# google/sentencepiece

Hardware: AMD Instinct MI355X
Metric: sentences/sec EncodeBatch, 32k unigram, MI355X (higher is better)
Workload: dtype u8 text -> i32 ids; f64 add / f32 store in the Viterbi relax

## Files before the change

### sentencepiece_amd/csrc/api.cc

```cpp
#include <hip/hip_runtime.h>

#include <cstdio>
#include <cstdlib>
#include <fcntl.h>
#include <sys/mman.h>
#include <sys/stat.h>
#include <sys/syscall.h>
#include <unistd.h>

#include <algorithm>
#include <cmath>
#include <condition_variable>
#include <cstring>
#include <fstream>
#include <functional>
#include <map>
#include <memory>
#include <mutex>
#include <thread>
#include <new>
#include <sstream>
#include <atomic>
#include <chrono>
#include <string>
// ... 650 lines not shown
  HIP_OR_RETURN(h, ws->d_tmp_off.Reserve(n + 1));
  HIP_OR_RETURN(h, ws->d_tile_sums.Reserve((n + kScanTile - 1) / kScanTile + 2));
  HIP_OR_RETURN(h, ws->d_big_list.Reserve((n + 63) / 64 + 1));
  if (!d_status) { HIP_OR_RETURN(h, ws->d_sent_status.Reserve(n)); d_status = ws->d_sent_status.p; }
  uint32_t *const class_lists = ws->d_lists.p;
  uint32_t *const over_list = class_lists + static_cast<size_t>(kMaxClasses - 1) * n;
  uint32_t *const hard_lists = class_lists + static_cast<size_t>(kMaxClasses) * n;
  uint32_t *const long_list = class_lists + static_cast<size_t>(2 * kMaxClasses) * n;
  uint32_t *const retry_lists[2] = {long_list + n, long_list + 2 * n};
  uint32_t *const left_lists[3] = {long_list + 3 * n, long_list + (3 + static_cast<size_t>(kMaxClasses)) * n,
                                   long_list + (3 + 2 * static_cast<size_t>(kMaxClasses)) * n};
  uint32_t *const gen_lists = long_list + (3 + 3 * static_cast<size_t>(kMaxClasses)) * n;
  uint64_t expand = (h->dev.flags & kNfCompressSp) || !(h->dev.flags & kNfEscapeWs) ? 1 : 3;
  if ((h->dev.flags & kNfCompressSp) && (h->dev.flags & kNfByteFallback)) expand = 2;
  uint64_t arena_need = expand * text_bytes + (10 + static_cast<uint64_t>(h->dev.n_prefix + h->dev.n_suffix)) * n + 4096;
  const bool prof = h->profiling;
  if (prof) HIP_OR_RETURN(h, EnsureEvents(ws));
  const uint32_t n32 = static_cast<uint32_t>(n);
  const int wide = h->n_cu * 8;
  const bool fast_ok = StreamFastEligible(h->dev.flags) && !h->no_fast;
  const bool uds = (h->dev.flags & kNfHasUserDefined) != 0;
  uint32_t rcaps[kMaxClasses] = {0};
  for (int c = 0; c < ncls; ++c) rcaps[c] = cls[c].rcap;
  rcaps[ncls - 1] = cls[ncls - 1].rcap;
  const uint64_t max_raw = (0x7FFFFF00ull - 16) / h->dev.expand_max;
  auto record = [&](int slot, int which) -> hipError_t {
    return prof ? hipEventRecord(ws->ev[slot][which], stream) : hipSuccess;
  };
  auto scan_compact = [&]() -> int {
    ScanArgs sa{ws->d_counts.p, n32, ws->d_tile_sums.p, d_id_offsets};
    const uint32_t tiles = (n32 + kScanTile - 1) / kScanTile;
    HIP_OR_RETURN(h, LaunchScan(sa, static_cast<int>(tiles < static_cast<uint32_t>(wide) ? tiles : wide), stream));
    const uint32_t big = (n < 65536 || text_bytes > 160ull * n) ? h->compact_big : 0u;
    CompactArgs pa{ws->d_arena.p, ws->d_tmp_off.p, ws->d_counts.p, d_id_offsets, d_ids, d_ids ? ids_capacity : 0, n32, &ws->d_ctrl->status, h->compact_staged,
                   big, ws->d_big_list.p, &ws->d_ctrl->big_count[0]};
    const uint64_t cblocks = (n + 63) / 64;
    const uint64_t cgrid = cblocks < static_cast<uint64_t>(h->n_cu) * 32 ? cblocks : static_cast<uint64_t>(h->n_cu) * 32;
    HIP_OR_RETURN(h, LaunchCompact(pa, static_cast<int>(cgrid), stream));
    if (big) HIP_OR_RETURN(h, LaunchCompactBig(pa, h->n_cu * 4, stream));
    HIP_OR_RETURN(h, hipMemcpyAsync(ws->h_ctrl, ws->d_ctrl, offsetof(Ctrl, total_ids), hipMemcpyDeviceToHost, stream));
    HIP_OR_RETURN(h, hipMemcpyAsync(&ws->h_ctrl->total_ids, d_id_offsets + n, sizeof(uint64_t), hipMemcpyDeviceToHost, stream));
    HIP_OR_RETURN(h, hipStreamSynchronize(stream));
    return kOk;
  };
  uint64_t arena_cap_limit = 0;
  if (h->arena_first && arena_need > h->arena_first) { arena_need = h->arena_first; arena_cap_limit = h->arena_first; }
  const uint64_t arena_reserve = (h->arena_first || ws->reserve_text_bytes <= text_bytes) ? 0 :
      expand * ws->reserve_text_bytes + (10 + static_cast<uint64_t>(h->dev.n_prefix + h->dev.n_suffix)) * (ws->reserve_n > n ? ws->reserve_n : n) + 4096;
  for (int attempt = 0; attempt < 4; ++attempt) {
    HIP_OR_RETURN(h, ws->d_arena.Reserve(arena_need > arena_reserve ? arena_need : arena_reserve));
    if (spans) HIP_OR_RETURN(h, ws->d_arena_tb.Reserve(ws->d_arena.cap));
    if (prof) HIP_OR_RETURN(h, hipEventRecord(ws->ev[kNumSlots][0], stream));
    HIP_OR_RETURN(h, hipMemsetAsync(ws->d_ctrl, 0, sizeof(Ctrl), stream));
    HIP_OR_RETURN(h, hipMemsetAsync(d_status, 0, n, stream));
    for (bool &u : ws->slot_used) u = false;
    const bool direct = word_ok && any_word && h->word_form == 3 && !h->no_direct && streaming;
    uint32_t known[kMaxClasses] = {0};
    uint32_t gen_known[kMaxClasses] = {0};
    uint64_t gen_total = 0;
    if (!direct) {
      if (int rc = RunClassify(h, ws, d_offsets, n32, stream, scanned ? d_text : nullptr, text_bytes, scanned ? gen_lists : nullptr); rc != kOk) return rc;
      HIP_OR_RETURN(h, hipMemcpyAsync(ws->h_ctrl->list_counts, ws->d_ctrl->list_counts,
                                      sizeof(ws->h_ctrl->list_counts) + sizeof(ws->h_ctrl->gen_counts),
                                      hipMemcpyDeviceToHost, stream));
      HIP_OR_RETURN(h, hipStreamSynchronize(stream));
      for (int c = 0; c < ncls; ++c) { known[c] = ws->h_ctrl->list_counts[c]; gen_known[c] = ws->h_ctrl->gen_counts[c]; gen_total += gen_known[c]; }
    } else {
      known[0] = n32;
    }
    EncodeArgs a{};
    a.dev = h->dev; a.text = d_text; a.offs = d_offsets;
// ... 286 lines not shown
        }
        wa.total_main = tile_base;
        wa.q = &ws->d_ctrl->q[qi];
        wa.stats = &ws->d_ctrl->stats[kStatsPerClass * slot];
        wa.left_lists = out_lists;
        wa.left_counts = d_out_counts;
        wa.left2_lists = out2_lists;
        wa.left2_counts = d_out2_counts;
        wa.dyn_tag = ws->d_dyn_tag.p;
        wa.dyn_ent = ws->d_dyn_ent.p;
        wa.dyn_list = ws->d_dyn_list.p;
        wa.dyn_count = &ws->d_ctrl->dyn_count;
        wa.dyn_mask = h->dyn_slots - 1u;
        wa.dyn_cap = h->dyn_list_cap;
        wa.resume = ws->d_resume.p;
        wa.ids16 = (h->model.pieces.size() <= 65536 && !h->no_ids16) ? 1u : 0u;
        snprintf(ws->slot_name[slot], sizeof(ws->slot_name[slot]), "%s",
                 wform ? (wa.ids16 ? (mode == 2 ? "EncodeWordWaveAgainKernel<true>" : mode == 1 ? "EncodeWordWaveCollectKernel<true>" : "EncodeWordWaveKernel<true>")
                                   : (mode == 2 ? "EncodeWordWaveAgainKernel<false>" : mode == 1 ? "EncodeWordWaveCollectKernel<false>" : "EncodeWordWaveKernel<false>"))
                       : mode == 3 ? "EncodeWordDpKernel" : mode == 2 ? "EncodeWordAgainKernel" : mode == 1 ? "EncodeWordCollectKernel" : "EncodeWordKernel");
        HIP_OR_RETURN(h, record(slot, 0));
        if (wform) HIP_OR_RETURN(h, LaunchEncodeWordWave(mode, wa, static_cast<int>(grid), waves, WordWaveLdsBytes(waves), stream));
        else HIP_OR_RETURN(h, LaunchEncodeWord(mode, wa, static_cast<int>(grid), waves, WordLdsBytes(waves, dp), stream));
        HIP_OR_RETURN(h, record(slot, 1));
        ws->slot_used[slot] = true;
        return kOk;
      };
      auto read_counts = [&]() -> int {
        HIP_OR_RETURN(h, hipMemcpyAsync(ws->h_ctrl->left_counts, ws->d_ctrl->left_counts, sizeof(ws->h_ctrl->left_counts) + sizeof(uint32_t),
                                        hipMemcpyDeviceToHost, stream));
        HIP_OR_RETURN(h, hipStreamSynchronize(stream));
// ... 111 lines not shown
      Profile &p = ws->prof;
      p = Profile();
      p.n = kNumSlots;
      for (int c = 0; c < kNumSlots; ++c) {
        if (!ws->slot_used[c]) continue;
        memcpy(p.name[c], ws->slot_name[c], sizeof(p.name[c]));
        HIP_OR_RETURN(h, hipEventElapsedTime(&p.kernel_ms[c], ws->ev[c][0], ws->ev[c][1]));
        const unsigned long long *s = &ws->h_ctrl->stats[kStatsPerClass * c];
        p.sentences[c] = s[0];
        p.raw_bytes[c] = s[1];
        p.ids[c] = s[2];
        for (int k = 0; k < 5; ++k) p.cycles[c][k] = s[3 + k];
      }
      p.path[0] = ws->h_ctrl->side.n_backlog; p.path[1] = ws->h_ctrl->side.over_count; p.path[2] = ws->h_ctrl->side.long_count;
      p.path[3] = ws->h_ctrl->side.n_failed;
      HIP_OR_RETURN(h, hipEventElapsedTime(&p.total_ms, ws->ev[kNumSlots][0], ws->ev[kNumSlots][1]));
      std::lock_guard<std::mutex> l(h->mu);
      h->prof = p;
    }
    if (total_ids) *total_ids = ws->h_ctrl->total_ids;
    if (n_failed) *n_failed = ws->h_ctrl->side.n_failed;
    if (ws->h_ctrl->total_ids > ids_capacity || !d_ids) {
      if (ws->h_ctrl->total_ids == 0) return kOk;
      return Fail(h, kResourceExhausted, "ids_capacity is too small");
    }
    if (spans && ws->h_ctrl->total_ids > 0) {
      const uint64_t total = ws->h_ctrl->total_ids;
      HIP_OR_RETURN(h, ws->d_tok_begin.Reserve(total));
      CompactArgs pa{ws->d_arena_tb.p, ws->d_tmp_off.p, ws->d_counts.p, d_id_offsets, ws->d_tok_begin.p, total, n32, nullptr, h->compact_staged,
                     h->compact_big, ws->d_big_list.p, &ws->d_ctrl->big_count[1]};
      const uint64_t cblocks = (n + 63) / 64;
      const uint64_t cgrid = cblocks < static_cast<uint64_t>(h->n_cu) * 32 ? cblocks : static_cast<uint64_t>(h->n_cu) * 32;
      HIP_OR_RETURN(h, LaunchCompact(pa, static_cast<int>(cgrid), stream));
      if (h->compact_big) HIP_OR_RETURN(h, LaunchCompactBig(pa, h->n_cu * 4, stream));
      HIP_OR_RETURN(h, hipMemsetAsync(&ws->d_ctrl->status, 0, sizeof(uint32_t), stream));
      HIP_OR_RETURN(h, hipMemsetAsync(ws->d_ctrl->align_counts, 0, sizeof(ws->d_ctrl->align_counts), stream));
      HIP_OR_RETURN(h, hipMemsetAsync(&ws->d_ctrl->side.long_count, 0, sizeof(uint32_t), stream));
      AlignArgs base{};
      base.dev = h->dev; base.text = d_text; base.offs = d_offsets;
      base.id_offs = d_id_offsets; base.tok_begin = ws->d_tok_begin.p; base.begin = d_begin; base.end = d_end;
      base.nbegin = d_nbegin; base.nend = d_nbegin ? d_nend : nullptr;
      base.status = &ws->d_ctrl->status; base.list_cap = n32;
      bool prev = false;
      int c_staged = 0;
      while (c_staged < ncls && cls[c_staged].rcap <= kMaxStagedRaw) ++c_staged;
// ... 1694 lines not shown
  snprintf(out, cap, "%s", h->prof.name[slot]);
  return static_cast<int>(strlen(h->prof.name[slot]));
}

int spmx_last_profile(const spmx_handle *h, float *kernel_ms, uint64_t *sentences, uint64_t *raw_bytes, uint64_t *ids,
                      uint64_t *bytes, uint64_t *path, float *total_ms) {
  if (!h) return 0;
  const Profile &p = h->prof;
  for (int c = 0; c < p.n; ++c) {
    if (kernel_ms) kernel_ms[c] = p.kernel_ms[c];
    if (sentences) sentences[c] = p.sentences[c];
    if (raw_bytes) raw_bytes[c] = p.raw_bytes[c];
    if (ids) ids[c] = p.ids[c];
    if (bytes) bytes[c] = p.raw_bytes[c] + 16 * p.sentences[c] + 4 * p.ids[c];
  }
  if (path) for (int k = 0; k < 4; ++k) path[k] = p.path[k];
  if (total_ms) *total_ms = p.total_ms;
  return p.n;
}

}
```

### sentencepiece_amd/csrc/kernels.h

```cpp
#ifndef SPMX_KERNELS_H_
#define SPMX_KERNELS_H_

#ifndef SPMX_WAVE_API
#include "wave.h"
#endif
#include <math.h>

#include "dev.h"

namespace spmx {

enum : uint32_t {
  kStArenaOverflow = 1u << 0,
  kStTooLong = 1u << 1,
  kStInternal = 1u << 2,
};
enum : uint32_t { kSsOk = 0, kSsResourceExhausted = 8, kSsOutOfRange = 11, kSsInternal = 13 };

constexpr int kMaxClasses = 8;

struct StreamClass {
  uint32_t rcap;
  uint32_t tcap;
  uint32_t lane_shift;
// ... 53 lines not shown
  uint32_t no_char_norm;
  StreamClass cls[kMaxClasses];
  uint32_t *left_lists;
  uint32_t *left_counts;
  uint32_t *left2_lists;
  uint32_t *left2_counts;
  unsigned long long *dyn_tag;
  U4 *dyn_ent;
  uint32_t *dyn_list;
  uint32_t *dyn_count;
  uint32_t dyn_mask;
  uint32_t dyn_cap;
  U4 *resume;
  uint32_t ids16;
  uint32_t direct;
  const uint32_t *list;
  const uint32_t *list_count;
  uint32_t *next_list;
  uint32_t *next_count;
  uint32_t rcap, ncap;
};

constexpr int kStatsPerClass = 8;
constexpr uint32_t kTokEnd = 0x8000u;

SPMX_DEVICE uint32_t DartsOffset(uint32_t u) { return (u >> 10) << ((u & (1u << 9)) >> 6); }

SPMX_DEVICE int OneCharLenDev(uint32_t c) {
  const uint32_t h = c >> 4;
  return h < 12 ? 1 : (h < 14 ? 2 : (h == 14 ? 3 : 4));
// ... 1106 lines not shown
```

### sentencepiece_amd/csrc/kernels_word.h

```cpp
#ifndef SPMX_KERNELS_WORD_H_
#define SPMX_KERNELS_WORD_H_

namespace spmx {

constexpr uint32_t kWordMaskBytes = 18u * 16u + 32u;
constexpr uint32_t kWordLdsShared = kWordMaskBytes + kWordHotSlots * 16u;
constexpr uint32_t kWordStage = 8;
constexpr uint32_t kWordDpPos = 18;
constexpr int kWordDpMax = 4;
constexpr uint32_t kDynMaxIds = 8;
constexpr uint32_t kDynMaxWide = 16;
constexpr uint32_t kDynFirstUnk = 0x100u, kDynLastUnk = 0x200u, kDynWide = 0x400u;
constexpr uint32_t kDynProbes = 24;
enum { kWmPlain = 0, kWmCollect = 1, kWmDyn = 2 };
SPMX_DEVICE unsigned long long DynTag(uint32_t k0, uint32_t k1, uint32_t k2, uint32_t k3) {
  const uint32_t h1 = HashWordKey(k0, k1, k2, k3);
  const unsigned long long t = (static_cast<unsigned long long>(h1) << 32) | UallHash2(k0, k1, k2, k3, h1);
  return t | 1ull;
}
SPMX_HD inline uint32_t WordLdsPerWave(bool dp) {
  return 64u * kWordStage * 4u + (dp ? 64u * (kWordDpPos * 8u + 20u) : 0u);
}
SPMX_HD inline uint32_t WordLdsBytes(uint32_t waves, bool dp) { return kWordLdsShared + waves * WordLdsPerWave(dp); }

// ... 416 lines not shown
    if (!got) break;
    c = wv::shfl(c, 0); first = wv::shfl(first, 0); ucnt = wv::shfl(ucnt, 0);
    const unsigned long long c0 = wv::clock();
    const uint32_t *list = a.lists + static_cast<uint64_t>(c) * a.n;
    const bool have = static_cast<uint32_t>(lane) < ucnt;
    uint32_t sid = 0;
    uint64_t beg = 0, l64 = 0;
    if (have) {
      sid = list[first + static_cast<uint32_t>(lane)];
      beg = a.offs[sid];
      l64 = a.offs[sid + 1] - beg;
    }
    const bool mine = have && !a.cls[c].general && l64 < (1ull << 30) && beg + l64 + 20u <= text_end;
    const int len = mine ? static_cast<int>(l64) : 0;
    const int cap = mine ? len + 1 : 0;
    const int room = (mine && MODE != kWmDyn) ? (cap + n_extra + 3 + 3) & ~3 : 0;
    int total = 0;
    const int excl = wave_excl_scan(room, lane, &total);
    unsigned long long base = 0;
    if (lane == 0 && total > 0) base = wv::atomic_add(a.arena_head, static_cast<unsigned long long>(total + 3));
    base = (static_cast<unsigned long long>(wv::shfl(static_cast<uint32_t>(base >> 32), 0)) << 32) |
           wv::shfl(static_cast<uint32_t>(base), 0);
    const bool overflow = base + static_cast<unsigned long long>(total + 3) > a.arena_cap;
    if (overflow && lane == 0) wv::atomic_or(a.status, kStArenaOverflow);
    base = (base + 3ull) & ~3ull;
    const int at = excl + d.n_prefix;
    const int shift = (4 - (at & 3)) & 3;
    int32_t *slot = a.arena + base + static_cast<unsigned long long>(excl + shift) + d.n_prefix;
    WordResume rs{0, 0, 0.f};
    if (MODE == kWmDyn && mine) {
      slot = a.arena + a.tmp_off[sid] + d.n_prefix;
      const U4 r = a.resume[sid];
      rs.p = static_cast<int>(r.x); rs.n = static_cast<int>(r.y); rs.B = wv::bits_to_float(r.z);
    }
    int steps = 0;
    int n = uni_word_lane<DP, MODE, H16>(a, a.text, beg, len, slot, cap, T, mine && !overflow, &steps, &rs);
    const unsigned long long c1 = wv::clock();
    if (overflow) n = -1;
    const bool done = mine && n >= 0;
    if (done) {
      if (H16) {
        uint16_t *s16 = reinterpret_cast<uint16_t *>(slot);
        for (int x = 0; x < d.n_prefix; ++x) s16[x - d.n_prefix] = static_cast<uint16_t>(d.prefix_ids[x]);
        for (int x = 0; x < d.n_suffix; ++x) s16[n + x] = static_cast<uint16_t>(d.suffix_ids[x]);
        a.tmp_off[sid] = kTmpOffHalf | (2ull * static_cast<unsigned long long>(slot - a.arena) - static_cast<unsigned long long>(d.n_prefix));
      } else {
        for (int x = 0; x < d.n_prefix; ++x) slot[x - d.n_prefix] = d.prefix_ids[x];
        for (int x = 0; x < d.n_suffix; ++x) slot[n + x] = d.suffix_ids[x];
        a.tmp_off[sid] = static_cast<unsigned long long>(slot - d.n_prefix - a.arena);
      }
      a.counts[sid] = static_cast<uint32_t>(n + n_extra);
    }
    const bool left = have && !done;
    if (left) a.counts[sid] = 0u;
    if (MODE == kWmCollect) {
      const bool again = left && n == -2;
      const bool gone = left && !again;
      if (again) {
        a.resume[sid] = U4{static_cast<uint32_t>(rs.p), static_cast<uint32_t>(rs.n), wv::float_to_bits(rs.B), 0u};
        a.tmp_off[sid] = static_cast<unsigned long long>(slot - d.n_prefix - a.arena);
      }
      append_lanes(wv::ballot(again), again, sid, a.left_lists + static_cast<uint64_t>(c) * a.n, &a.left_counts[c], lane);
      append_lanes(wv::ballot(gone), gone, sid, a.left2_lists + static_cast<uint64_t>(c) * a.n, &a.left2_counts[c], lane);
    } else {
      append_lanes(wv::ballot(left), left, sid, a.left_lists + static_cast<uint64_t>(c) * a.n, &a.left_counts[c], lane);
    }
    if (done) { ++tc.n_sent; tc.n_raw += static_cast<unsigned long long>(len); tc.n_ids += static_cast<unsigned long long>(n + n_extra); }
    tc.n_trips += static_cast<unsigned long long>(steps);
    tc.cyc[2] += c1 - c0;
    tc.cyc[3] += wv::clock() - c1;
  }
  if (a.stats) {
    unsigned long long v[3] = {tc.n_sent, tc.n_raw, tc.n_ids};
    for (int k = 0; k < 3; ++k) {
      uint64_t tot = 0;
// ... 533 lines not shown
```

### sentencepiece_amd/csrc/kernels_wordwave.h

```cpp
#ifndef SPMX_KERNELS_WORDWAVE_H_
#define SPMX_KERNELS_WORDWAVE_H_

namespace spmx {

constexpr uint32_t kWwRing = 4096u;
constexpr uint32_t kWwRingPad = 32u;
constexpr uint32_t kWwUnits = kWwRing / 16u;
constexpr uint32_t kWwMaskBytes = (kWwUnits + 4u) * 2u + 8u;
constexpr uint32_t kWwRecs = 128u + 512u;
constexpr uint32_t kWwMaxLen = 65536u;
constexpr uint32_t kWwPerWave = kWwRing + kWwRingPad + kWwMaskBytes + kWwRecs * 4u + 64u * 16u + 64u * 8u + 5u * 64u * 4u;
static_assert(kWwPerWave % 16u == 0u, "per-wave LDS blocks keep 16-byte alignment");
constexpr uint32_t kWwAgain = 1u, kWwGone = 2u;
constexpr uint32_t kWwKeyMaskBytes = 640u;
constexpr uint32_t kWwShared = kWwKeyMaskBytes + kWordHotSlots * 16u + kUallBuckets * 2u;
SPMX_HD constexpr bool kWwHotIn(int mode) { return mode == 2; }
SPMX_HD inline uint32_t WordWaveLdsBytes(uint32_t waves) { return kWwShared + waves * kWwPerWave; }

struct __attribute__((packed, aligned(2))) U64H { uint32_t lo, hi; };

SPMX_DEVICE uint32_t space_mask16(const Q4 &v) {
  auto m4 = [](uint32_t z) -> uint32_t { return (((z >> 7) & 0x01010101u) * 0x10204080u) >> 28; };
  return m4(space_flags(v.x)) | (m4(space_flags(v.y)) << 4) | (m4(space_flags(v.z)) << 8) | (m4(space_flags(v.w)) << 12);
}
// ... 37 lines not shown
      masks[2 * lane] = Q4{m(0), m(1), m(2), m(3)};
      masks[2 * lane + 1] = Q4{kWordKeyPad & ~m(0), kWordKeyPad & ~m(1), kWordKeyPad & ~m(2), kWordKeyPad & ~m(3)};
    }
    if (kWwHotIn(MODE)) for (uint32_t k = static_cast<uint32_t>(lane); k < kWordHotSlots; k += 64u) hot[k] = d.uhot2[k];
    for (uint32_t k = static_cast<uint32_t>(lane); k < kUallBuckets; k += 64u) disp[k] = d.udisp[k];
    wv::sync();
  }
  const U4 *__restrict__ uall = d.uall;
  const uint32_t mall = d.uall_mask;
  const bool perfect = d.uall_perfect != 0u;
  const int n_extra = d.n_prefix + d.n_suffix;
  const bool keep_ws = (d.flags & kNfRemoveExtraWs) == 0;
  const bool any_word = (d.flags & kNfWordLocalNorm) != 0;
  const uint64_t tbase = reinterpret_cast<uint64_t>(a.text);
  WaveCounters tc;
  WwStage SA{}, SB{};
  uint32_t dyn_warm = 0u;
  for (;;) {
    const unsigned long long cs = wv::clock();
    uint32_t c = 0, first = 0, ucnt = 0, got = 0;
    if (lane == 0) got = next_tile(a, &c, &first, &ucnt) ? 1u : 0u;
    got = wv::shfl(got, 0);
    if (!got) break;
    c = wv::shfl(c, 0); first = wv::shfl(first, 0); ucnt = wv::shfl(ucnt, 0);
    const bool direct = a.direct != 0u;
    const uint32_t *list = a.lists ? a.lists + static_cast<uint64_t>(c) * a.n : nullptr;
    const bool have = static_cast<uint32_t>(lane) < ucnt;
    uint32_t sid = 0;
    uint64_t beg = 0, l64 = 0;
    if (have) {
      sid = list ? list[first + static_cast<uint32_t>(lane)] : first + static_cast<uint32_t>(lane);
      beg = a.offs[sid];
      l64 = a.offs[sid + 1] - beg;
    }
    uint32_t cl = c;
    if (direct) {
      cl = a.n_classes - 1u;
      for (int k = static_cast<int>(a.n_classes) - 2; k >= 0; --k) if (l64 <= a.cls[k].rcap) cl = static_cast<uint32_t>(k);
    }
    const bool mine = have && !a.cls[cl].general && l64 <= kWwMaxLen;
    const int cap = mine ? static_cast<int>(l64) + 1 : 0;
    const int room = (mine && MODE != kWmDyn) ? (cap + n_extra + 3 + 3) & ~3 : 0;
    int total = 0;
    const int excl = wave_excl_scan(room, lane, &total);
    unsigned long long base = 0;
    if (lane == 0 && total > 0) base = wv::atomic_add(a.arena_head, static_cast<unsigned long long>(total + 3));
    base = (static_cast<unsigned long long>(wv::shfl(static_cast<uint32_t>(base >> 32), 0)) << 32) |
           wv::shfl(static_cast<uint32_t>(base), 0);
    const bool overflow = base + static_cast<unsigned long long>(total + 3) > a.arena_cap;
    if (overflow && lane == 0) wv::atomic_or(a.status, kStArenaOverflow);
    base = (base + 3ull) & ~3ull;
    const int at = excl + d.n_prefix;
    const int shift = (4 - (at & 3)) & 3;
    int32_t *slot = a.arena + base + static_cast<unsigned long long>(excl + shift) + d.n_prefix;
    uint32_t p0 = 0u, n0 = 0u, x0 = 0u;
    if (MODE == kWmDyn && mine) {
      slot = a.arena + a.tmp_off[sid] + d.n_prefix;
      const U4 rs = a.resume[sid];
      const float bf0 = wv::bits_to_float(rs.z);
      if (rs.x < l64 && rs.y <= rs.x && bf0 >= 0.f && bf0 < 16777216.f) { p0 = rs.x; n0 = rs.y; x0 = static_cast<uint32_t>(bf0); }
    }
    const bool work = mine && !overflow;
    const uint32_t len = work ? static_cast<uint32_t>(l64) - p0 : 0u;
    beg += p0;
    const uint32_t begmod = static_cast<uint32_t>((tbase + beg) & 15ull);
    const uint32_t nun = len ? (begmod + len + 15u) >> 4 : 0u;
    const uint32_t pu_incl = wv::scan_add(nun);
    const uint32_t pu = pu_incl - nun;
    const uint32_t U = wv::read_lane(pu_incl, 63);
    {
      const uint32_t start = pu * 16u + begmod;
      const uint64_t ua = tbase + beg - begmod;
      const uint64_t so = static_cast<uint64_t>(slot - a.arena);
      sent[lane] = U4{start, start + len, static_cast<uint32_t>(so), static_cast<uint32_t>(so >> 32)};
      sent_ua[lane] = U2{static_cast<uint32_t>(ua), static_cast<uint32_t>(ua >> 32)};
      s_nids[lane] = n0;
      s_stat[lane] = 0u;
      s_first[lane] = 0xFFFFFFFFu;
      if (MODE == kWmDyn) { s_n0[lane] = n0; s_x0[lane] = x0; }
    }
    wv::sync();
    const unsigned long long c0 = wv::clock();
    tc.cyc[0] += c0 - cs;
    const uint32_t rounds = (U + 63u) >> 6;
    auto issue = [&](uint32_t q, Q4 *v, uint32_t *jq) __attribute__((always_inline)) {
      const uint32_t u = q * 64u + static_cast<uint32_t>(lane);
      const bool ok = u < U;
      int lo = 0;
#pragma unroll
// ... 29 lines not shown
      const uint32_t hi = s.y - ub < 16u ? s.y - ub : 16u;
      const uint32_t vm = ((1u << hi) - 1u) & ~((1u << lo) - 1u);
      uint32_t before = (spm << 1) | ((!firstu && prevb == 0x20u) ? 1u : 0u);
      if (firstu) before |= 1u << lo;
      if (keep_ws && ok) {
        const uint32_t lead = firstu ? (spm >> lo) & 1u : 0u;
        const uint32_t dbl = spm & before & vm & ~(firstu ? 1u << lo : 0u);
        const uint32_t trail = (s.y - ub <= 16u) ? (spm >> (hi - 1u)) & 1u : 0u;
        if (lead | dbl | trail) wv::lds_atomic_or(&s_stat[j], kWwGone);
      }
      return ok ? (~spm & before & vm) : 0u;
    };

    SA.cnt = 0u; SB.cnt = 0u;
    uint32_t carry_j = 0xFFFFFFFFu, carry_x = 0u, carry_n = 0u, carry_unk = 0u;
    unsigned long long steps = 0;

    auto stageA = [&](uint32_t qbase, uint32_t qcnt, WwStage &S) __attribute__((always_inline)) {
      S.cnt = qcnt;
      const uint32_t l32 = static_cast<uint32_t>(lane);
      const bool valid = l32 < qcnt;
      const uint32_t rec = recq[qbase + (valid ? l32 : (qcnt ? qcnt - 1u : 0u))];
      const uint32_t P = rec & 0x03FFFFFFu, j = rec >> 26;
      const uint32_t s_end = sent[j].y;
      const Q4U w = *reinterpret_cast<const Q4U *>(ring + (P & (kWwRing - 1u)));
      const U64H sm = *reinterpret_cast<const U64H *>(smask + ((P >> 4) & (kWwUnits - 1u)));
      const uint64_t bits = (static_cast<uint64_t>(sm.hi) << 32 | sm.lo) >> (P & 15u);
      const uint32_t rem = s_end - P;
      uint32_t L = static_cast<uint32_t>(wv::ffs64(bits | (1ull << 17))) - 1u;
      if (L > rem) L = rem;
// ... 137 lines not shown
      if (MODE == kWmDyn) {
        const uint32_t pl = wv::lane_up1(lastunk, 0u);
        const bool prev_unk = head ? (cont && carry_unk != 0u) : pl != 0u;
        if (hitd && (dn & kDynFirstUnk) && prev_unk) skip = 1u;
      }
      const uint32_t cntd = dn & 0xFFu;
      if (MODE == kWmDyn) {
        const uint32_t pl = wv::lane_up1(lastunk, 0u);
        const bool prev_unk = head ? (cont && carry_unk != 0u) : pl != 0u;
        if (word && hitd && cntd == 0u && prev_unk) gone = true;
      }
      const uint32_t cnt = !word ? 0u : (hitd ? cntd - skip : (hit ? (id1 != 0xFFFFFFFFu ? 2u : 1u) : 0u));
      const uint32_t packed = (x << 12) | cnt;
      const uint32_t Sc = wv::scan_add(packed);
      const uint32_t E = Sc - packed;
      const uint32_t hE = wv::scan_max(head ? E : 0u);
      const uint32_t rel = E - hE;
      uint32_t xb = rel >> 12, nb = rel & 0xFFFu;
      uint32_t n0j = 0u;
      if (MODE == kWmDyn) n0j = s_n0[j];
      if (cont) { xb += carry_x; nb += carry_n; }
      else if (MODE == kWmDyn) { xb += s_x0[j]; nb += n0j; }
      {
        const int lv = static_cast<int>(S.cnt - 1u);
        carry_j = wv::read_lane(j, lv);
        carry_x = wv::read_lane(xb + x, lv);
        carry_n = wv::read_lane(nb + cnt, lv);
        carry_unk = wv::read_lane(lastunk, lv);
      }
      if (word && hit && !(xb < (1u << 24) && static_cast<float>(xb) < lim)) gone = true;
      const U4 sj = sent[j];
      if (MODE == kWmDyn && word && hit && nb + cnt > sj.y - sj.x + 1u + n0j) gone = true;
      const bool emit = word && hit && !gone;
      const uint64_t so = static_cast<uint64_t>(sj.w) << 32 | sj.z;
      if (emit && !hitd) {
        if (H16) {
          uint16_t *q = reinterpret_cast<uint16_t *>(a.arena + so) + nb;
          q[0] = static_cast<uint16_t>(id0);
          if (cnt == 2u) q[1] = static_cast<uint16_t>(id1);
        } else {
          int32_t *q = a.arena + so + nb;
          q[0] = static_cast<int32_t>(id0);
          if (cnt == 2u) q[1] = static_cast<int32_t>(id1);
        }
      }
      if (MODE == kWmDyn && wv::any(emit && hitd)) {
        const bool wide = (dn & kDynWide) != 0u;
        auto idc = [&](uint32_t t) __attribute__((always_inline)) -> uint32_t {
          const uint32_t di[8] = {dia.x, dia.y, dia.z, dia.w, dib.x, dib.y, dib.z, dib.w};
          if (wide) return t < 16u ? (di[(t >> 1) & 7u] >> (16u * (t & 1u))) & 0xFFFFu : 0u;
          return t < 8u ? di[t & 7u] : 0u;
        };
        const uint32_t maxc = wv::read_lane(wv::scan_max((emit && hitd) ? cnt : 0u), 63);
#pragma unroll
        for (uint32_t t = 0; t < kDynMaxWide; ++t) {
          if (t >= maxc) break;
          if (emit && hitd && t < cnt) {
            const uint32_t id = skip ? idc(t + 1u) : idc(t);
            if (H16) reinterpret_cast<uint16_t *>(a.arena + so)[nb + t] = static_cast<uint16_t>(id);
            else (a.arena + so)[nb + t] = static_cast<int32_t>(id);
          }
        }
      }
      const uint32_t jnext = wv::lane_down1(word ? j : 0xFFFFFFFEu, 0xFFFFFFFEu);
      if (word && jnext != j) s_nids[j] = nb + cnt;
      if (wv::any(gone || miss)) {
        if (gone) wv::lds_atomic_or(&s_stat[j], kWwGone);
        if (miss) { wv::lds_atomic_or(&s_stat[j], kWwAgain); wv::lds_atomic_min(&s_first[j], P); }
        wv::sync();
        if (MODE == kWmCollect) {
          const bool wr = miss && s_first[j] == P;
          const uint32_t sidj = wv::shfl(sid, static_cast<int>(j));
          if (wr) a.resume[sidj] = U4{P - sj.x, nb, wv::float_to_bits(static_cast<float>(xb)), 0u};
        }
      }
// ... 54 lines not shown
        wv::sync();
        if (l32 < left) recq[l32] = v0;
        if (l32 + 64u < left) recq[l32 + 64u] = v1;
      }
      qn = left;
      wv::sync();
      ws_cur = ws_next;
      j_cur = j_next;
    }
    stageB(SB);
    SB.cnt = 0u;
    wv::sync();
    const unsigned long long c1 = wv::clock();
    const uint32_t st = s_stat[lane];
    const int n = static_cast<int>(s_nids[lane]);
    const bool done = work && st == 0u;
    if (done) {
      if (H16) {
        uint16_t *s16 = reinterpret_cast<uint16_t *>(slot);
        for (int x = 0; x < d.n_prefix; ++x) s16[x - d.n_prefix] = static_cast<uint16_t>(d.prefix_ids[x]);
        for (int x = 0; x < d.n_suffix; ++x) s16[n + x] = static_cast<uint16_t>(d.suffix_ids[x]);
        a.tmp_off[sid] = kTmpOffHalf | (2ull * static_cast<unsigned long long>(slot - a.arena) - static_cast<unsigned long long>(d.n_prefix));
      } else {
        for (int x = 0; x < d.n_prefix; ++x) slot[x - d.n_prefix] = d.prefix_ids[x];
        for (int x = 0; x < d.n_suffix; ++x) slot[n + x] = d.suffix_ids[x];
        a.tmp_off[sid] = static_cast<unsigned long long>(slot - d.n_prefix - a.arena);
      }
      a.counts[sid] = static_cast<uint32_t>(n + n_extra);
    }
    const bool left = have && !done;
    if (left) a.counts[sid] = 0u;
    auto hand_on = [&](bool pred, uint32_t *lists, uint32_t *counts) __attribute__((always_inline)) {
      if (!direct) { append_lanes(wv::ballot(pred), pred, sid, lists + static_cast<uint64_t>(c) * a.n, &counts[c], lane); return; }
      if (!wv::any(pred)) return;
      for (uint32_t k = 0; k < a.n_classes; ++k) {
        const bool pk = pred && cl == k;
        append_lanes(wv::ballot(pk), pk, sid, lists + static_cast<uint64_t>(k) * a.n, &counts[k], lane);
      }
    };
    if (MODE == kWmCollect) {
      const bool again = left && work && st == kWwAgain;
      const bool gonel = left && !again;
      if (again) a.tmp_off[sid] = static_cast<unsigned long long>(slot - d.n_prefix - a.arena);
      const uint32_t ca = direct ? 0u : c;
      append_lanes(wv::ballot(again), again, sid, a.left_lists + static_cast<uint64_t>(ca) * a.n, &a.left_counts[ca], lane);
      hand_on(gonel, a.left2_lists, a.left2_counts);
    } else {
      hand_on(left, a.left_lists, a.left_counts);
    }
    if (done) { ++tc.n_sent; tc.n_raw += static_cast<unsigned long long>(len); tc.n_ids += static_cast<unsigned long long>(n + n_extra); }
    tc.n_trips += steps;
    tc.cyc[2] += c1 - c0;
    tc.cyc[3] += wv::clock() - c1;
  }
  if (a.stats) {
    unsigned long long v[3] = {tc.n_sent, tc.n_raw, tc.n_ids};
    for (int k = 0; k < 3; ++k) {
      uint64_t tot = 0;
// ... 13 lines not shown
```

### sentencepiece_amd/processor.py

```python
import ctypes as C
import os

import numpy as np

from . import _capi

_PYEXT = [False, None]


def _pyext():
    if _PYEXT[0] is False:
        try:
            from . import _spmx_py
            _PYEXT[1] = _spmx_py
        except ImportError:
            _PYEXT[1] = None
        _PYEXT[0] = True
    return _PYEXT[1]

_OK = 0
_RESOURCE_EXHAUSTED = 8


class SentencePieceProcessor:
# ... 994 lines not shown
        tot = C.c_float(0)
        k = self._lib.spmx_last_profile(self._h, ms.ctypes.data, sent.ctypes.data, raw.ctypes.data, ids.ctypes.data,
                                        byt.ctypes.data, path.ctypes.data, C.byref(tot))
        cyc = np.zeros(80, dtype=np.uint64)
        self._lib.spmx_last_phase_cycles(self._h, cyc.ctypes.data)
        names = []
        for c in range(k):
            buf = C.create_string_buffer(64)
            self._lib.spmx_last_profile_name(self._h, c, buf, 64)
            names.append(buf.value.decode())
        return dict(classes=[dict(kernel=names[c], kernel_ms=float(ms[c]), sentences=int(sent[c]), raw_bytes=int(raw[c]),
                                  ids=int(ids[c]), bytes=int(byt[c]),
                                  phase_cycles=dict(zip(("load", "normalize", "segment", "emit", "search_trips"),
                                                        (int(x) for x in cyc[5 * c:5 * c + 5]))))
                             for c in range(k)],
                    path=dict(backlog=int(path[0]), overflow=int(path[1]), long=int(path[2]), failed=int(path[3])),
                    total_ms=float(tot.value))
```

Measured before the change: 2.232 billion.

## Pack word-wave output ids contiguously in arena with fixed direct region

In direct mode the word-wave kernel now places each sentence's ids at an offset computed from the text offsets, inside a pre-reserved arena region, instead of taking per-wave atomic allocations. Slots are packed with 16-bit granularity when ids16 is set, so there is no padding. Emitted ids are written at a running per-wave offset, and the dynamic/resume mode copies the partial output into the new packed slot. The aim is fewer atomics, less arena space and tighter data for the later compact pass, at the cost of a copy on resume and new overflow checks. It also adds arena-retry reporting and resets the big_count counters.

Result: faster. 2.398 billion, median of 6 (+7.4%).

```diff
diff --git a/sentencepiece_amd/csrc/api.cc b/sentencepiece_amd/csrc/api.cc
--- a/sentencepiece_amd/csrc/api.cc
+++ b/sentencepiece_amd/csrc/api.cc
@@ -688,6 +688,14 @@
   uint64_t expand = (h->dev.flags & kNfCompressSp) || !(h->dev.flags & kNfEscapeWs) ? 1 : 3;
   if ((h->dev.flags & kNfCompressSp) && (h->dev.flags & kNfByteFallback)) expand = 2;
   uint64_t arena_need = expand * text_bytes + (10 + static_cast<uint64_t>(h->dev.n_prefix + h->dev.n_suffix)) * n + 4096;
+  const bool direct = word_ok && any_word && h->word_form == 3 && !h->no_direct && streaming;
+  const bool ids16 = h->model.pieces.size() <= 65536 && !h->no_ids16;
+  uint64_t direct_region = 0;
+  if (direct) {
+    const uint64_t units = text_bytes + (1 + static_cast<uint64_t>(h->dev.n_prefix + h->dev.n_suffix)) * n;
+    direct_region = ((ids16 ? (units + 1) / 2 : units) + 7) & ~static_cast<uint64_t>(3);
+    arena_need += direct_region;
+  }
   const bool prof = h->profiling;
   if (prof) HIP_OR_RETURN(h, EnsureEvents(ws));
   const uint32_t n32 = static_cast<uint32_t>(n);
@@ -706,6 +714,7 @@
     const uint32_t tiles = (n32 + kScanTile - 1) / kScanTile;
     HIP_OR_RETURN(h, LaunchScan(sa, static_cast<int>(tiles < static_cast<uint32_t>(wide) ? tiles : wide), stream));
     const uint32_t big = (n < 65536 || text_bytes > 160ull * n) ? h->compact_big : 0u;
+    if (big) HIP_OR_RETURN(h, hipMemsetAsync(&ws->d_ctrl->big_count[0], 0, sizeof(uint32_t), stream));
     CompactArgs pa{ws->d_arena.p, ws->d_tmp_off.p, ws->d_counts.p, d_id_offsets, d_ids, d_ids ? ids_capacity : 0, n32, &ws->d_ctrl->status, h->compact_staged,
                    big, ws->d_big_list.p, &ws->d_ctrl->big_count[0]};
     const uint64_t cblocks = (n + 63) / 64;
@@ -720,7 +729,8 @@
   uint64_t arena_cap_limit = 0;
   if (h->arena_first && arena_need > h->arena_first) { arena_need = h->arena_first; arena_cap_limit = h->arena_first; }
   const uint64_t arena_reserve = (h->arena_first || ws->reserve_text_bytes <= text_bytes) ? 0 :
-      expand * ws->reserve_text_bytes + (10 + static_cast<uint64_t>(h->dev.n_prefix + h->dev.n_suffix)) * (ws->reserve_n > n ? ws->reserve_n : n) + 4096;
+      expand * ws->reserve_text_bytes + (10 + static_cast<uint64_t>(h->dev.n_prefix + h->dev.n_suffix)) * (ws->reserve_n > n ? ws->reserve_n : n) + 4096 +
+      (direct ? (ws->reserve_text_bytes + (1 + static_cast<uint64_t>(h->dev.n_prefix + h->dev.n_suffix)) * (ws->reserve_n > n ? ws->reserve_n : n)) / (ids16 ? 2 : 1) + 8 : 0);
   for (int attempt = 0; attempt < 4; ++attempt) {
     HIP_OR_RETURN(h, ws->d_arena.Reserve(arena_need > arena_reserve ? arena_need : arena_reserve));
     if (spans) HIP_OR_RETURN(h, ws->d_arena_tb.Reserve(ws->d_arena.cap));
@@ -728,7 +738,6 @@
     HIP_OR_RETURN(h, hipMemsetAsync(ws->d_ctrl, 0, sizeof(Ctrl), stream));
     HIP_OR_RETURN(h, hipMemsetAsync(d_status, 0, n, stream));
     for (bool &u : ws->slot_used) u = false;
-    const bool direct = word_ok && any_word && h->word_form == 3 && !h->no_direct && streaming;
     uint32_t known[kMaxClasses] = {0};
     uint32_t gen_known[kMaxClasses] = {0};
     uint64_t gen_total = 0;
@@ -1045,7 +1054,8 @@
         wa.dyn_mask = h->dyn_slots - 1u;
         wa.dyn_cap = h->dyn_list_cap;
         wa.resume = ws->d_resume.p;
-        wa.ids16 = (h->model.pieces.size() <= 65536 && !h->no_ids16) ? 1u : 0u;
+        wa.ids16 = ids16 ? 1u : 0u;
+        wa.arena_first = (direct && mode != 2) ? direct_region : 0u;
         snprintf(ws->slot_name[slot], sizeof(ws->slot_name[slot]), "%s",
                  wform ? (wa.ids16 ? (mode == 2 ? "EncodeWordWaveAgainKernel<true>" : mode == 1 ? "EncodeWordWaveCollectKernel<true>" : "EncodeWordWaveKernel<true>")
                                    : (mode == 2 ? "EncodeWordWaveAgainKernel<false>" : mode == 1 ? "EncodeWordWaveCollectKernel<false>" : "EncodeWordWaveKernel<false>"))
@@ -1187,6 +1197,7 @@
       }
       p.path[0] = ws->h_ctrl->side.n_backlog; p.path[1] = ws->h_ctrl->side.over_count; p.path[2] = ws->h_ctrl->side.long_count;
       p.path[3] = ws->h_ctrl->side.n_failed;
+      p.path[4] = static_cast<uint64_t>(attempt);
       HIP_OR_RETURN(h, hipEventElapsedTime(&p.total_ms, ws->ev[kNumSlots][0], ws->ev[kNumSlots][1]));
       std::lock_guard<std::mutex> l(h->mu);
       h->prof = p;
@@ -1202,6 +1213,7 @@
       HIP_OR_RETURN(h, ws->d_tok_begin.Reserve(total));
       CompactArgs pa{ws->d_arena_tb.p, ws->d_tmp_off.p, ws->d_counts.p, d_id_offsets, ws->d_tok_begin.p, total, n32, nullptr, h->compact_staged,
                      h->compact_big, ws->d_big_list.p, &ws->d_ctrl->big_count[1]};
+      if (h->compact_big) HIP_OR_RETURN(h, hipMemsetAsync(&ws->d_ctrl->big_count[1], 0, sizeof(uint32_t), stream));
       const uint64_t cblocks = (n + 63) / 64;
       const uint64_t cgrid = cblocks < static_cast<uint64_t>(h->n_cu) * 32 ? cblocks : static_cast<uint64_t>(h->n_cu) * 32;
       HIP_OR_RETURN(h, LaunchCompact(pa, static_cast<int>(cgrid), stream));
@@ -2926,7 +2938,7 @@
     if (ids) ids[c] = p.ids[c];
     if (bytes) bytes[c] = p.raw_bytes[c] + 16 * p.sentences[c] + 4 * p.ids[c];
   }
-  if (path) for (int k = 0; k < 4; ++k) path[k] = p.path[k];
+  if (path) for (int k = 0; k < 5; ++k) path[k] = p.path[k];
   if (total_ms) *total_ms = p.total_ms;
   return p.n;
 }
diff --git a/sentencepiece_amd/csrc/kernels.h b/sentencepiece_amd/csrc/kernels.h
--- a/sentencepiece_amd/csrc/kernels.h
+++ b/sentencepiece_amd/csrc/kernels.h
@@ -91,6 +91,7 @@
   U4 *resume;
   uint32_t ids16;
   uint32_t direct;
+  uint64_t arena_first;
   const uint32_t *list;
   const uint32_t *list_count;
   uint32_t *next_list;
diff --git a/sentencepiece_amd/csrc/kernels_word.h b/sentencepiece_amd/csrc/kernels_word.h
--- a/sentencepiece_amd/csrc/kernels_word.h
+++ b/sentencepiece_amd/csrc/kernels_word.h
@@ -454,7 +454,7 @@
     const bool mine = have && !a.cls[c].general && l64 < (1ull << 30) && beg + l64 + 20u <= text_end;
     const int len = mine ? static_cast<int>(l64) : 0;
     const int cap = mine ? len + 1 : 0;
-    const int room = (mine && MODE != kWmDyn) ? (cap + n_extra + 3 + 3) & ~3 : 0;
+    const int room = mine ? (cap + n_extra + 3 + 3) & ~3 : 0;
     int total = 0;
     const int excl = wave_excl_scan(room, lane, &total);
     unsigned long long base = 0;
@@ -469,9 +469,18 @@
     int32_t *slot = a.arena + base + static_cast<unsigned long long>(excl + shift) + d.n_prefix;
     WordResume rs{0, 0, 0.f};
     if (MODE == kWmDyn && mine) {
-      slot = a.arena + a.tmp_off[sid] + d.n_prefix;
       const U4 r = a.resume[sid];
       rs.p = static_cast<int>(r.x); rs.n = static_cast<int>(r.y); rs.B = wv::bits_to_float(r.z);
+      const uint64_t t = a.tmp_off[sid];
+      const uint64_t src = ((t & kTmpOffHalf) ? (t & ~kTmpOffHalf) : (H16 ? 2ull * t : t)) + static_cast<uint64_t>(d.n_prefix);
+      if (!overflow && rs.n > 0 && rs.n <= cap) {
+        if (H16) {
+          const uint16_t *f16 = reinterpret_cast<const uint16_t *>(a.arena) + src;
+          for (int x = 0; x < rs.n; ++x) reinterpret_cast<uint16_t *>(slot)[x] = f16[x];
+        } else {
+          for (int x = 0; x < rs.n; ++x) slot[x] = a.arena[src + x];
+        }
+      }
     }
     int steps = 0;
     int n = uni_word_lane<DP, MODE, H16>(a, a.text, beg, len, slot, cap, T, mine && !overflow, &steps, &rs);
@@ -498,7 +507,8 @@
       const bool gone = left && !again;
       if (again) {
         a.resume[sid] = U4{static_cast<uint32_t>(rs.p), static_cast<uint32_t>(rs.n), wv::float_to_bits(rs.B), 0u};
-        a.tmp_off[sid] = static_cast<unsigned long long>(slot - d.n_prefix - a.arena);
+        a.tmp_off[sid] = H16 ? kTmpOffHalf | (2ull * static_cast<unsigned long long>(slot - a.arena) - static_cast<unsigned long long>(d.n_prefix))
+                             : static_cast<unsigned long long>(slot - d.n_prefix - a.arena);
       }
       append_lanes(wv::ballot(again), again, sid, a.left_lists + static_cast<uint64_t>(c) * a.n, &a.left_counts[c], lane);
       append_lanes(wv::ballot(gone), gone, sid, a.left2_lists + static_cast<uint64_t>(c) * a.n, &a.left2_counts[c], lane);
diff --git a/sentencepiece_amd/csrc/kernels_wordwave.h b/sentencepiece_amd/csrc/kernels_wordwave.h
--- a/sentencepiece_amd/csrc/kernels_wordwave.h
+++ b/sentencepiece_amd/csrc/kernels_wordwave.h
@@ -75,6 +75,8 @@
   const bool any_word = (d.flags & kNfWordLocalNorm) != 0;
   const uint64_t tbase = reinterpret_cast<uint64_t>(a.text);
   WaveCounters tc;
+  if (MODE != kWmDyn && a.arena_first != 0u && wv::block_id() == 0 && wv::wave_in_block() == 0 && lane == 0)
+    wv::atomic_add(a.arena_head, static_cast<unsigned long long>(a.arena_first));
   WwStage SA{}, SB{};
   uint32_t dyn_warm = 0u;
   for (;;) {
@@ -100,27 +102,41 @@
       for (int k = static_cast<int>(a.n_classes) - 2; k >= 0; --k) if (l64 <= a.cls[k].rcap) cl = static_cast<uint32_t>(k);
     }
     const bool mine = have && !a.cls[cl].general && l64 <= kWwMaxLen;
-    const int cap = mine ? static_cast<int>(l64) + 1 : 0;
-    const int room = (mine && MODE != kWmDyn) ? (cap + n_extra + 3 + 3) & ~3 : 0;
-    int total = 0;
-    const int excl = wave_excl_scan(room, lane, &total);
-    unsigned long long base = 0;
-    if (lane == 0 && total > 0) base = wv::atomic_add(a.arena_head, static_cast<unsigned long long>(total + 3));
-    base = (static_cast<unsigned long long>(wv::shfl(static_cast<uint32_t>(base >> 32), 0)) << 32) |
-           wv::shfl(static_cast<uint32_t>(base), 0);
-    const bool overflow = base + static_cast<unsigned long long>(total + 3) > a.arena_cap;
-    if (overflow && lane == 0) wv::atomic_or(a.status, kStArenaOverflow);
-    base = (base + 3ull) & ~3ull;
-    const int at = excl + d.n_prefix;
-    const int shift = (4 - (at & 3)) & 3;
-    int32_t *slot = a.arena + base + static_cast<unsigned long long>(excl + shift) + d.n_prefix;
     uint32_t p0 = 0u, n0 = 0u, x0 = 0u;
+    uint64_t src0 = 0;
     if (MODE == kWmDyn && mine) {
-      slot = a.arena + a.tmp_off[sid] + d.n_prefix;
+      const uint64_t t = a.tmp_off[sid];
+      src0 = ((t & kTmpOffHalf) ? (t & ~kTmpOffHalf) : (H16 ? 2ull * t : t)) + static_cast<uint64_t>(d.n_prefix);
       const U4 rs = a.resume[sid];
       const float bf0 = wv::bits_to_float(rs.z);
       if (rs.x < l64 && rs.y <= rs.x && bf0 >= 0.f && bf0 < 16777216.f) { p0 = rs.x; n0 = rs.y; x0 = static_cast<uint32_t>(bf0); }
     }
+    const bool fixed = direct && list == nullptr && MODE != kWmDyn;
+    const uint64_t room = !have ? 0ull : static_cast<uint64_t>(n_extra) + ((fixed || mine) ? l64 + 1ull : 0ull);
+    uint64_t rtotal = 0;
+    wave_excl_scan64(room, lane, &rtotal);
+    uint64_t base = 0;
+    bool overflow;
+    if (fixed) {
+      const uint64_t o0 = a.offs[0];
+      base = (static_cast<uint64_t>(wv::shfl(static_cast<uint32_t>(beg >> 32), 0)) << 32 | wv::shfl(static_cast<uint32_t>(beg), 0)) - o0 +
+             static_cast<uint64_t>(first) * static_cast<uint64_t>(1 + n_extra);
+      const uint64_t end32 = H16 ? (base + rtotal + 1ull) / 2ull : base + rtotal;
+      overflow = end32 > a.arena_cap || end32 > a.arena_first;
+    } else {
+      const uint64_t need = H16 ? (rtotal + 1ull) / 2ull : rtotal;
+      unsigned long long b32 = 0;
+      if (lane == 0 && rtotal > 0) b32 = wv::atomic_add(a.arena_head, static_cast<unsigned long long>(need + 3ull));
+      b32 = (static_cast<unsigned long long>(wv::shfl(static_cast<uint32_t>(b32 >> 32), 0)) << 32) |
+            wv::shfl(static_cast<uint32_t>(b32), 0);
+      overflow = b32 + need + 3ull > a.arena_cap;
+      b32 = (b32 + 3ull) & ~3ull;
+      base = H16 ? 2ull * b32 : b32;
+    }
+    if (overflow && lane == 0) wv::atomic_or(a.status, kStArenaOverflow);
+    const uint64_t rend = base + rtotal;
+    const uint64_t sbase = base + static_cast<uint64_t>(lane) * static_cast<uint64_t>(n_extra) + static_cast<uint64_t>(d.n_prefix) +
+                           wv::scan_add(n0);
     const bool work = mine && !overflow;
     const uint32_t len = work ? static_cast<uint32_t>(l64) - p0 : 0u;
     beg += p0;
@@ -132,8 +148,7 @@
     {
       const uint32_t start = pu * 16u + begmod;
       const uint64_t ua = tbase + beg - begmod;
-      const uint64_t so = static_cast<uint64_t>(slot - a.arena);
-      sent[lane] = U4{start, start + len, static_cast<uint32_t>(so), static_cast<uint32_t>(so >> 32)};
+      sent[lane] = U4{start, start + len, static_cast<uint32_t>(sbase), static_cast<uint32_t>(sbase >> 32)};
       sent_ua[lane] = U2{static_cast<uint32_t>(ua), static_cast<uint32_t>(ua >> 32)};
       s_nids[lane] = n0;
       s_stat[lane] = 0u;
@@ -193,6 +208,7 @@
 
     SA.cnt = 0u; SB.cnt = 0u;
     uint32_t carry_j = 0xFFFFFFFFu, carry_x = 0u, carry_n = 0u, carry_unk = 0u;
+    uint32_t carry_t = 0u;
     unsigned long long steps = 0;
 
     auto stageA = [&](uint32_t qbase, uint32_t qcnt, WwStage &S) __attribute__((always_inline)) {
@@ -360,6 +376,8 @@
       const uint32_t packed = (x << 12) | cnt;
       const uint32_t Sc = wv::scan_add(packed);
       const uint32_t E = Sc - packed;
+      const uint32_t T = carry_t + (E & 0xFFFu);
+      carry_t += wv::read_lane(Sc, 63) & 0xFFFu;
       const uint32_t hE = wv::scan_max(head ? E : 0u);
       const uint32_t rel = E - hE;
       uint32_t xb = rel >> 12, nb = rel & 0xFFFu;
@@ -377,15 +395,16 @@
       if (word && hit && !(xb < (1u << 24) && static_cast<float>(xb) < lim)) gone = true;
       const U4 sj = sent[j];
       if (MODE == kWmDyn && word && hit && nb + cnt > sj.y - sj.x + 1u + n0j) gone = true;
+      const uint64_t so = (static_cast<uint64_t>(sj.w) << 32 | sj.z) + T;
+      if (word && hit && so + cnt > rend) gone = true;
       const bool emit = word && hit && !gone;
-      const uint64_t so = static_cast<uint64_t>(sj.w) << 32 | sj.z;
       if (emit && !hitd) {
         if (H16) {
-          uint16_t *q = reinterpret_cast<uint16_t *>(a.arena + so) + nb;
+          uint16_t *q = reinterpret_cast<uint16_t *>(a.arena) + so;
           q[0] = static_cast<uint16_t>(id0);
           if (cnt == 2u) q[1] = static_cast<uint16_t>(id1);
         } else {
-          int32_t *q = a.arena + so + nb;
+          int32_t *q = a.arena + so;
           q[0] = static_cast<int32_t>(id0);
           if (cnt == 2u) q[1] = static_cast<int32_t>(id1);
         }
@@ -403,8 +422,8 @@
           if (t >= maxc) break;
           if (emit && hitd && t < cnt) {
             const uint32_t id = skip ? idc(t + 1u) : idc(t);
-            if (H16) reinterpret_cast<uint16_t *>(a.arena + so)[nb + t] = static_cast<uint16_t>(id);
-            else (a.arena + so)[nb + t] = static_cast<int32_t>(id);
+            if (H16) reinterpret_cast<uint16_t *>(a.arena)[so + t] = static_cast<uint16_t>(id);
+            else a.arena[so + t] = static_cast<int32_t>(id);
           }
         }
       }
@@ -489,19 +508,58 @@
     const unsigned long long c1 = wv::clock();
     const uint32_t st = s_stat[lane];
     const int n = static_cast<int>(s_nids[lane]);
-    const bool done = work && st == 0u;
+    const uint64_t sstart = base + static_cast<uint64_t>(lane) * static_cast<uint64_t>(n_extra) +
+                            static_cast<uint64_t>(wv::scan_add(static_cast<uint32_t>(n)) - static_cast<uint32_t>(n));
+    const bool done = work && st == 0u && sstart + static_cast<uint64_t>(n + n_extra) <= rend;
+    const unsigned long long toff = H16 ? (kTmpOffHalf | sstart) : sstart;
     if (done) {
       if (H16) {
-        uint16_t *s16 = reinterpret_cast<uint16_t *>(slot);
-        for (int x = 0; x < d.n_prefix; ++x) s16[x - d.n_prefix] = static_cast<uint16_t>(d.prefix_ids[x]);
-        for (int x = 0; x < d.n_suffix; ++x) s16[n + x] = static_cast<uint16_t>(d.suffix_ids[x]);
-        a.tmp_off[sid] = kTmpOffHalf | (2ull * static_cast<unsigned long long>(slot - a.arena) - static_cast<unsigned long long>(d.n_prefix));
+        uint16_t *s16 = reinterpret_cast<uint16_t *>(a.arena) + sstart;
+        for (int x = 0; x < d.n_prefix; ++x) s16[x] = static_cast<uint16_t>(d.prefix_ids[x]);
+        for (int x = 0; x < d.n_suffix; ++x) s16[d.n_prefix + n + x] = static_cast<uint16_t>(d.suffix_ids[x]);
       } else {
-        for (int x = 0; x < d.n_prefix; ++x) slot[x - d.n_prefix] = d.prefix_ids[x];
-        for (int x = 0; x < d.n_suffix; ++x) slot[n + x] = d.suffix_ids[x];
-        a.tmp_off[sid] = static_cast<unsigned long long>(slot - d.n_prefix - a.arena);
-      }
+        int32_t *s32 = a.arena + sstart;
+        for (int x = 0; x < d.n_prefix; ++x) s32[x] = d.prefix_ids[x];
+        for (int x = 0; x < d.n_suffix; ++x) s32[d.n_prefix + n + x] = d.suffix_ids[x];
+      }
+      a.tmp_off[sid] = toff;
       a.counts[sid] = static_cast<uint32_t>(n + n_extra);
+    }
+    if (MODE == kWmDyn) {
+      const uint32_t cn = done ? n0 : 0u;
+      const uint32_t ci = wv::scan_add(cn);
+      const uint32_t cx = ci - cn;
+      const uint32_t ctot = wv::read_lane(ci, 63);
+      const uint64_t dst0 = sstart + static_cast<uint64_t>(d.n_prefix);
+      for (uint32_t k0 = 0; k0 < ctot; k0 += 256u) {
+        uint32_t v[4];
+        uint64_t to[4];
+#pragma unroll
+        for (uint32_t u = 0; u < 4u; ++u) {
+          const uint32_t k = k0 + 64u * u + static_cast<uint32_t>(lane);
+          int lo = 0;
+#pragma unroll
+          for (int step = 32; step >= 1; step >>= 1) {
+            const uint32_t pv = wv::shfl(cx, lo + step);
+            if (pv <= k) lo += step;
+          }
+          const uint32_t r = k - wv::shfl(cx, lo);
+          const uint64_t from = (static_cast<uint64_t>(wv::shfl(static_cast<uint32_t>(src0 >> 32), lo)) << 32 |
+                                 wv::shfl(static_cast<uint32_t>(src0), lo)) + r;
+          to[u] = (static_cast<uint64_t>(wv::shfl(static_cast<uint32_t>(dst0 >> 32), lo)) << 32 |
+                   wv::shfl(static_cast<uint32_t>(dst0), lo)) + r;
+          v[u] = 0u;
+          if (k < ctot) v[u] = H16 ? reinterpret_cast<const uint16_t *>(a.arena)[from] : static_cast<uint32_t>(a.arena[from]);
+        }
+#pragma unroll
+        for (uint32_t u = 0; u < 4u; ++u) {
+          const uint32_t k = k0 + 64u * u + static_cast<uint32_t>(lane);
+          if (k < ctot) {
+            if (H16) reinterpret_cast<uint16_t *>(a.arena)[to[u]] = static_cast<uint16_t>(v[u]);
+            else a.arena[to[u]] = static_cast<int32_t>(v[u]);
+          }
+        }
+      }
     }
     const bool left = have && !done;
     if (left) a.counts[sid] = 0u;
@@ -516,7 +574,7 @@
     if (MODE == kWmCollect) {
       const bool again = left && work && st == kWwAgain;
       const bool gonel = left && !again;
-      if (again) a.tmp_off[sid] = static_cast<unsigned long long>(slot - d.n_prefix - a.arena);
+      if (again) a.tmp_off[sid] = toff;
       const uint32_t ca = direct ? 0u : c;
       append_lanes(wv::ballot(again), again, sid, a.left_lists + static_cast<uint64_t>(ca) * a.n, &a.left_counts[ca], lane);
       hand_on(gonel, a.left2_lists, a.left2_counts);
diff --git a/sentencepiece_amd/processor.py b/sentencepiece_amd/processor.py
--- a/sentencepiece_amd/processor.py
+++ b/sentencepiece_amd/processor.py
@@ -1032,5 +1032,6 @@
                                   phase_cycles=dict(zip(("load", "normalize", "segment", "emit", "search_trips"),
                                                         (int(x) for x in cyc[5 * c:5 * c + 5]))))
                              for c in range(k)],
-                    path=dict(backlog=int(path[0]), overflow=int(path[1]), long=int(path[2]), failed=int(path[3])),
+                    path=dict(backlog=int(path[0]), overflow=int(path[1]), long=int(path[2]), failed=int(path[3]),
+                              arena_retries=int(path[4])),
                     total_ms=float(tot.value))
```
